# aim-uofa/DiverGen

Measured on AMD Instinct MI355X. Metric: images/sec (node) Swin-L CenterNet2 LVIS 1024px, higher is better.
Workload: dtype bf16; 1 GPU; CenterNet2 Swin-L-22k-384, 1024x1024, 2 images/GPU, 1453 classes, GPU copy-paste + fwd + bwd + fused clip/AdamW/EMA; configs/DiverGen_swinL.yaml; global_batch=2, parallelism=dp1

## Files before the change

### divergen_amd/csrc/gemm_k192.hip

```cpp
#include "gemm_common.h"

namespace {
constexpr int KW_BROWS = 192, KW_KT = 3;
constexpr int KW_BKT = KW_BROWS * 128;
constexpr int KW_B_BYTES = KW_KT * KW_BKT;
template <int AR> struct KwCfg { static constexpr int WAVES = 192 / AR, AKT = AR * 128, A_BYTES = KW_KT * AKT, RI = AR / 16, RQ = AR / 8; };
struct KwParams {
    GemmP g;
    int ntn, row_tiles, wg_per_xcd;
};

template <int MC, int AR>
__global__ __launch_bounds__(KwCfg<AR>::WAVES * 64, 1) void gemm_k192_kernel(KwParams K) {
    constexpr int KW_WAVES = KwCfg<AR>::WAVES, KW_AKT = KwCfg<AR>::AKT, KW_A_BYTES = KwCfg<AR>::A_BYTES, KW_AROWS = AR, RI = KwCfg<AR>::RI,
                  RQ = KwCfg<AR>::RQ;
    GemmP& P = K.g;
    g_fix_mode<MC>(P);
    extern __shared__ __attribute__((aligned(1024))) unsigned char lds_raw[];
    const int tid = threadIdx.x, l = tid & 63;
    const int w = __builtin_amdgcn_readfirstlane(tid >> 6);
    const int c = l & 15, g = l >> 4;
    const int xcd = blockIdx.x & 7, slot = blockIdx.x >> 3;
    const int panel = slot % K.ntn;
    const int full = K.wg_per_xcd / K.ntn, extra = K.wg_per_xcd - full * K.ntn;
    const int groups = 8 * (full + (panel < extra ? 1 : 0));
    const int wave_rank = ((slot / K.ntn) * 8 + xcd) * KW_WAVES + w, wave_count = groups * KW_WAVES;
    const int n0 = panel * KW_BROWS;

    const int rsub = l >> 3;
    const uint32_t lds0 = (uint32_t)(uintptr_t)(DGX_LDS unsigned char*)lds_raw;
    {
        const u32x4 rB = buf_rsrc(P.B, (uint32_t)((int64_t)P.N * P.ldb * 2));
        for (int idx = w; idx < KW_KT * 24; idx += KW_WAVES) {
            const int kt = idx / 24, q = idx - kt * 24;
            const int lc = (l & 7) ^ (((q & 1) << 2) | (rsub >> 1));
            const int n = n0 + 8 * q + rsub;
            const uint32_t voff = (uint32_t)(((int64_t)n * P.ldb + lc * 8) * 2);
            lds_load16(voff, rB, __builtin_amdgcn_readfirstlane(lds0 + (uint32_t)(kt * KW_BKT + q * 1024)), (uint32_t)kt * 128u);
        }
    }
    const uint32_t abase = __builtin_amdgcn_readfirstlane(lds0 + (uint32_t)(KW_B_BYTES + w * KW_A_BYTES));
    const u32x4 rA = buf_rsrc(P.A, (uint32_t)((int64_t)P.M * P.lda * 2));
    uint32_t lcq[RQ];
#pragma unroll
    for (int q = 0; q < RQ; ++q) lcq[q] = (uint32_t)(((l & 7) ^ (((q & 1) << 2) | (rsub >> 1))) * 16);
    auto issue_a = [&](int tile) {
        const int m0 = tile * KW_AROWS;
#pragma unroll
        for (int q = 0; q < RQ; ++q) {
            const int m = m0 + 8 * q + rsub;
            const uint32_t voff = m < P.M ? (uint32_t)((int64_t)m * P.lda * 2) + lcq[q] : BUF_OOB;
#pragma unroll
            for (int kt = 0; kt < KW_KT; ++kt) lds_load16(voff, rA, abase + (uint32_t)(kt * KW_AKT + q * 1024), (uint32_t)kt * 128u);
        }
    };
    u32x2 braw[12];
#pragma unroll
    for (int j = 0; j < 12; ++j) braw[j] = P.bias ? *reinterpret_cast<const u32x2*>(P.bias + n0 + 16 * j + 4 * g) : u32x2{0u, 0u};
    int tile = wave_rank;
    if (tile < K.row_tiles) issue_a(tile);
    wait_vmcnt<0>();
    __syncthreads();

    const int swz = (c >> 1) & 7;
    const uint32_t fa = (uint32_t)(c * 128 + ((g ^ swz) << 4));
    DGX_LDS const unsigned char* pa = lds_opaque((const unsigned char*)lds_raw + KW_B_BYTES + w * KW_A_BYTES + fa);
    DGX_LDS const unsigned char* pa1 = lds_opaque((const unsigned char*)lds_raw + KW_B_BYTES + w * KW_A_BYTES + (fa ^ 64u));
    DGX_LDS const unsigned char* pb = lds_opaque((const unsigned char*)lds_raw + fa);
    DGX_LDS const unsigned char* pb1 = lds_opaque((const unsigned char*)lds_raw + (fa ^ 64u));
    const bool even = (g & 1) == 0;

    int gn[6];
#pragma unroll
    for (int p = 0; p < 6; ++p) gn[p] = n0 + 16 * (2 * p + (even ? 0 : 1)) + 4 * (even ? g : g - 1);
    for (; tile < K.row_tiles; tile += wave_count) {
        u32x4 xpre[MC == 4 ? RI : 1][6];
        if constexpr (MC == 4) {
#pragma unroll
            for (int i = 0; i < RI; ++i) {
                const int gm = tile * KW_AROWS + 16 * i + c;
#pragma unroll
                for (int p = 0; p < 6; ++p) xpre[i][p] = *reinterpret_cast<const u32x4*>(P.aux + (int64_t)(gm < P.M ? gm : 0) * P.ldaux + gn[p]);
            }
        }
        f32x4 acc[RI][12];
#pragma unroll
        for (int i = 0; i < RI; ++i)
#pragma unroll
            for (int j = 0; j < 12; ++j) acc[i][j] = f32x4{0.f, 0.f, 0.f, 0.f};
#pragma unroll
        for (int kt = 0; kt < KW_KT; ++kt)
#pragma unroll
            for (int kh = 0; kh < 2; ++kh) {
                DGX_LDS const unsigned char* a_ = (kh ? pa1 : pa) + kt * KW_AKT;
                DGX_LDS const unsigned char* b_ = (kh ? pb1 : pb) + kt * KW_BKT;
                bf16x8 af[RI];
#pragma unroll
                for (int i = 0; i < RI; ++i) af[i] = *reinterpret_cast<DGX_LDS const bf16x8*>(a_ + 2048 * i);
#pragma unroll
                for (int j = 0; j < 12; ++j) {
                    const bf16x8 b = *reinterpret_cast<DGX_LDS const bf16x8*>(b_ + 2048 * j);
#pragma unroll
                    for (int i = 0; i < RI; ++i) acc[i][j] = mfma16(b, af[i], acc[i][j]);
                }
            }
        const int m0 = tile * KW_AROWS;
        const int next = tile + wave_count;
        wait_lgkm0();
        if (next < K.row_tiles) issue_a(next);
#pragma unroll
        for (int i = 0; i < RI; ++i) {
            const int gm = m0 + 16 * i + c;
            int64_t tok = 0;
            float sc = 1.0f;
            bool ok = gm < P.M;
            if (P.mode == 3 && ok) {
                int b = 0;
                tok = wm_row_token<int64_t, G_ORDERS>(P.map, (int64_t)gm, b);
                ok = tok >= 0;
                if (ok && P.scale) sc = P.scale[b];
            }
            u32x4 y[6];
#pragma unroll
            for (int p = 0; p < 6; ++p) {
                u32x2 pk[2];
#pragma unroll
                for (int h = 0; h < 2; ++h) {
                    const int j = 2 * p + h;
                    const f32x4 a = acc[i][j];
                    float bv[4];
                    g_bias4(braw[j], bv);
                    pk[h] = u32x2{pack_bf2(a[0] + bv[0], a[1] + bv[1]), pack_bf2(a[2] + bv[2], a[3] + bv[3])};
                }
                const u32x2 give = even ? pk[1] : pk[0];
                const u32x2 got = u32x2{(uint32_t)__shfl_xor((int)give[0], 16), (uint32_t)__shfl_xor((int)give[1], 16)};
                y[p] = even ? u32x4{pk[0][0], pk[0][1], got[0], got[1]} : u32x4{got[0], got[1], pk[1][0], pk[1][1]};
            }
            u32x4 xa[6], xb[6];
            if constexpr (MC == 4) {
#pragma unroll
                for (int p = 0; p < 6; ++p) { xa[p] = xpre[i][p]; xb[p] = xa[p]; }
            } else if (P.mode >= 3) {
#pragma unroll
                for (int p = 0; p < 6; ++p) {
                    xa[p] = u32x4{0u, 0u, 0u, 0u}; xb[p] = xa[p];
                    g_epi_prefetch(P, ok ? gm : 0, gn[p], ok ? tok : 0, xa[p], xb[p]);
                }
            }
            if (ok) {
#pragma unroll
                for (int p = 0; p < 6; ++p) g_epi_finish(P, gm, gn[p], y[p], tok, sc, xa[p], xb[p]);
            }
        }
        constexpr int NST = (MC == 1 || MC == 4) ? RI * 6 : MC == 2 ? RI * 12 : -1;
        if (NST >= 0 && m0 + KW_AROWS <= P.M) wait_vmcnt<(NST >= 0 ? NST : 0)>();
        else wait_vmcnt<0>();
    }
}

template <int MC, int AR>
int launch_k192(KwParams& K, hipStream_t st, int grid) {
    static bool once = false;
    const size_t sm = (size_t)KW_B_BYTES + (size_t)KwCfg<AR>::WAVES * KwCfg<AR>::A_BYTES;
    K.row_tiles = (K.g.M + AR - 1) / AR;
    if (!once) {
        (void)hipFuncSetAttribute((const void*)gemm_k192_kernel<MC, AR>, hipFuncAttributeMaxDynamicSharedMemorySize, (int)sm);
        once = true;
    }
    hipLaunchKernelGGL((gemm_k192_kernel<MC, AR>), dim3(grid), dim3(KwCfg<AR>::WAVES * 64), sm, st, K);
    return DGX_OK;
}
}

bool dgx_gemm_k192_takes(const GemmP& P) {
    return P.lda >= 192 && ((uintptr_t)P.A & 15) == 0 && ((uintptr_t)P.B & 15) == 0 && (P.lda & 7) == 0 && (P.ldb & 7) == 0;
}
int dgx_gemm_k192_launch(const GemmP& P0, hipStream_t st) {
    extern int dgx_get_reserved_cus(void);
    KwParams K;
    K.g = P0;
    K.ntn = P0.N / KW_BROWS;
    K.row_tiles = 0;
    K.wg_per_xcd = 32 - dgx_get_reserved_cus() / 8;
    if (P0.K != 192 || K.ntn < 1 || K.wg_per_xcd < K.ntn) return DGX_ERR_UNSUPPORTED;
    const int grid = 8 * K.wg_per_xcd;
    return g_with_mc(g_tail_mc(P0), [&](auto mc) {
        constexpr int v = decltype(mc)::value;
        if constexpr (v == 5) return (int)DGX_ERR_UNSUPPORTED;
        else if constexpr (v <= 1) return launch_k192<1, 32>(K, st, grid);
        else return launch_k192<v, 16>(K, st, grid);
    });
}
```

Measured before the change: 80.81 images/s.

## Load A fragments straight to registers with prefetch, bias in LDS, retune waves

Adds a register-resident A path: each wave loads its A fragments directly from global memory into VGPRs in MFMA layout, double-buffered by prefetching the next tile before the current compute. This drops the LDS staging of A and frees LDS. The bias moves from per-lane registers into a small shared LDS table, and wave counts per workgroup are chosen separately per epilogue mode and panel count. The costs are higher VGPR pressure from the prefetch buffers, and 16-wide A tiles replace 32-wide ones for some modes.

```diff
diff --git a/divergen_amd/csrc/gemm_k192.hip b/divergen_amd/csrc/gemm_k192.hip
--- a/divergen_amd/csrc/gemm_k192.hip
+++ b/divergen_amd/csrc/gemm_k192.hip
@@ -4,16 +4,27 @@
 constexpr int KW_BROWS = 192, KW_KT = 3;
 constexpr int KW_BKT = KW_BROWS * 128;
 constexpr int KW_B_BYTES = KW_KT * KW_BKT;
-template <int AR> struct KwCfg { static constexpr int WAVES = 192 / AR, AKT = AR * 128, A_BYTES = KW_KT * AKT, RI = AR / 16, RQ = AR / 8; };
+template <int AR, int WV> struct KwCfg { static constexpr int WAVES = WV, RI = AR / 16, NA = RI * KW_KT * 2; };
+
+template <int OFF> __device__ __forceinline__ u32x4 kw_load16(uint32_t voff, u32x4 rsrc) {
+    u32x4 r;
+    asm volatile("buffer_load_dwordx4 %0, %1, %2, 0 offen offset:%3" : "=v"(r) : "v"(voff), "s"(rsrc), "n"(OFF) : "memory");
+    return r;
+}
+template <int NA> __device__ __forceinline__ void kw_landed(u32x4 (&a)[NA]) {
+    static_assert(NA == 6 || NA == 12, "fragments per lane");
+    asm volatile("" : "+v"(a[0]), "+v"(a[1]), "+v"(a[2]), "+v"(a[3]), "+v"(a[4]), "+v"(a[5])::"memory");
+    if constexpr (NA == 12) asm volatile("" : "+v"(a[6]), "+v"(a[7]), "+v"(a[8]), "+v"(a[9]), "+v"(a[10]), "+v"(a[11])::"memory");
+}
 struct KwParams {
     GemmP g;
     int ntn, row_tiles, wg_per_xcd;
 };
 
-template <int MC, int AR>
-__global__ __launch_bounds__(KwCfg<AR>::WAVES * 64, 1) void gemm_k192_kernel(KwParams K) {
-    constexpr int KW_WAVES = KwCfg<AR>::WAVES, KW_AKT = KwCfg<AR>::AKT, KW_A_BYTES = KwCfg<AR>::A_BYTES, KW_AROWS = AR, RI = KwCfg<AR>::RI,
-                  RQ = KwCfg<AR>::RQ;
+template <int MC, int AR, int WV, bool LDSA>
+__global__ __launch_bounds__(WV * 64, 1) void gemm_k192_kernel(KwParams K) {
+    constexpr int KW_WAVES = WV, KW_AROWS = AR, RI = KwCfg<AR, WV>::RI, NA = KwCfg<AR, WV>::NA;
+    constexpr int KW_AKT = AR * 128, KW_A_BYTES = KW_KT * KW_AKT, RQ = AR / 8, KW_BIAS_OFF = KW_B_BYTES + (LDSA ? WV * KW_A_BYTES : 0);
     GemmP& P = K.g;
     g_fix_mode<MC>(P);
     extern __shared__ __attribute__((aligned(1024))) unsigned char lds_raw[];
@@ -39,41 +50,63 @@
             lds_load16(voff, rB, __builtin_amdgcn_readfirstlane(lds0 + (uint32_t)(kt * KW_BKT + q * 1024)), (uint32_t)kt * 128u);
         }
     }
-    const uint32_t abase = __builtin_amdgcn_readfirstlane(lds0 + (uint32_t)(KW_B_BYTES + w * KW_A_BYTES));
     const u32x4 rA = buf_rsrc(P.A, (uint32_t)((int64_t)P.M * P.lda * 2));
-    uint32_t lcq[RQ];
-#pragma unroll
-    for (int q = 0; q < RQ; ++q) lcq[q] = (uint32_t)(((l & 7) ^ (((q & 1) << 2) | (rsub >> 1))) * 16);
-    auto issue_a = [&](int tile) {
+    const uint32_t abase =__builtin_amdgcn_readfirstlane(lds0 + (uint32_t)(KW_B_BYTES + w * KW_A_BYTES));
+    auto issue_a_lds = [&](int tile) {
         const int m0 = tile * KW_AROWS;
 #pragma unroll
         for (int q = 0; q < RQ; ++q) {
             const int m = m0 + 8 * q + rsub;
-            const uint32_t voff = m < P.M ? (uint32_t)((int64_t)m * P.lda * 2) + lcq[q] : BUF_OOB;
+            const uint32_t lcq = (uint32_t)(((l & 7) ^ (((q & 1) << 2) | (rsub >> 1))) * 16);
+            const uint32_t voff = m < P.M ? (uint32_t)((int64_t)m * P.lda * 2) + lcq : BUF_OOB;
 #pragma unroll
             for (int kt = 0; kt < KW_KT; ++kt) lds_load16(voff, rA, abase + (uint32_t)(kt * KW_AKT + q * 1024), (uint32_t)kt * 128u);
         }
     };
-    u32x2 braw[12];
-#pragma unroll
-    for (int j = 0; j < 12; ++j) braw[j] = P.bias ? *reinterpret_cast<const u32x2*>(P.bias + n0 + 16 * j + 4 * g) : u32x2{0u, 0u};
+    auto issue_a = [&](int tile, u32x4(&a)[NA]) {
+        static_for<RI>([&](auto i_) {
+            constexpr int i = decltype(i_)::value;
+            const int m = tile * KW_AROWS + 16 * i + c;
+            const uint32_t voff = m < P.M ? (uint32_t)((int64_t)m * P.lda * 2) + (uint32_t)(g * 16) : BUF_OOB;
+            static_for<KW_KT * 2>([&](auto k_) {
+                constexpr int k = decltype(k_)::value;
+                a[i * KW_KT * 2 + k] = kw_load16<k * 64>(voff, rA);
+            });
+        });
+    };
+    if (tid < KW_BROWS / 2)
+        reinterpret_cast<uint32_t*>(lds_raw + KW_BIAS_OFF)[tid] = P.bias ? *reinterpret_cast<const uint32_t*>(P.bias + n0 + 2 * tid) : 0u;
     int tile = wave_rank;
-    if (tile < K.row_tiles) issue_a(tile);
-    wait_vmcnt<0>();
+    u32x4 an[NA];
+    if constexpr (LDSA) {
+        if (tile < K.row_tiles) issue_a_lds(tile);
+        wait_vmcnt<0>();
+    } else {
+        issue_a(tile, an);
+        wait_vmcnt<0>();
+        kw_landed(an);
+    }
     __syncthreads();
 
     const int swz = (c >> 1) & 7;
     const uint32_t fa = (uint32_t)(c * 128 + ((g ^ swz) << 4));
+    DGX_LDS const unsigned char* pb = lds_opaque((const unsigned char*)lds_raw + fa);
+    DGX_LDS const unsigned char* pb1 = lds_opaque((const unsigned char*)lds_raw + (fa ^ 64u));
     DGX_LDS const unsigned char* pa = lds_opaque((const unsigned char*)lds_raw + KW_B_BYTES + w * KW_A_BYTES + fa);
     DGX_LDS const unsigned char* pa1 = lds_opaque((const unsigned char*)lds_raw + KW_B_BYTES + w * KW_A_BYTES + (fa ^ 64u));
-    DGX_LDS const unsigned char* pb = lds_opaque((const unsigned char*)lds_raw + fa);
-    DGX_LDS const unsigned char* pb1 = lds_opaque((const unsigned char*)lds_raw + (fa ^ 64u));
+    DGX_LDS const unsigned char* pbias = lds_opaque((const unsigned char*)lds_raw + KW_BIAS_OFF + 8 * g);
     const bool even = (g & 1) == 0;
 
     int gn[6];
 #pragma unroll
     for (int p = 0; p < 6; ++p) gn[p] = n0 + 16 * (2 * p + (even ? 0 : 1)) + 4 * (even ? g : g - 1);
     for (; tile < K.row_tiles; tile += wave_count) {
+        u32x4 ac[NA];
+        if constexpr (!LDSA) {
+#pragma unroll
+            for (int q = 0; q < NA; ++q) ac[q] = an[q];
+            issue_a(tile + wave_count, an);
+        }
         u32x4 xpre[MC == 4 ? RI : 1][6];
         if constexpr (MC == 4) {
 #pragma unroll
@@ -83,6 +116,7 @@
                 for (int p = 0; p < 6; ++p) xpre[i][p] = *reinterpret_cast<const u32x4*>(P.aux + (int64_t)(gm < P.M ? gm : 0) * P.ldaux + gn[p]);
             }
         }
+        asm volatile("" ::: "memory");
         f32x4 acc[RI][12];
 #pragma unroll
         for (int i = 0; i < RI; ++i)
@@ -92,11 +126,13 @@
         for (int kt = 0; kt < KW_KT; ++kt)
 #pragma unroll
             for (int kh = 0; kh < 2; ++kh) {
-                DGX_LDS const unsigned char* a_ = (kh ? pa1 : pa) + kt * KW_AKT;
                 DGX_LDS const unsigned char* b_ = (kh ? pb1 : pb) + kt * KW_BKT;
                 bf16x8 af[RI];
 #pragma unroll
-                for (int i = 0; i < RI; ++i) af[i] = *reinterpret_cast<DGX_LDS const bf16x8*>(a_ + 2048 * i);
+                for (int i = 0; i < RI; ++i) {
+                    if constexpr (LDSA) af[i] = *reinterpret_cast<DGX_LDS const bf16x8*>((kh ? pa1 : pa) + kt * KW_AKT + 2048 * i);
+                    else af[i] = __builtin_bit_cast(bf16x8, ac[(i * KW_KT + kt) * 2 + kh]);
+                }
 #pragma unroll
                 for (int j = 0; j < 12; ++j) {
                     const bf16x8 b = *reinterpret_cast<DGX_LDS const bf16x8*>(b_ + 2048 * j);
@@ -105,9 +141,10 @@
                 }
             }
         const int m0 = tile * KW_AROWS;
-        const int next = tile + wave_count;
-        wait_lgkm0();
-        if (next < K.row_tiles) issue_a(next);
+        if constexpr (LDSA) {
+            wait_lgkm0();
+            if (tile + wave_count < K.row_tiles) issue_a_lds(tile + wave_count);
+        }
 #pragma unroll
         for (int i = 0; i < RI; ++i) {
             const int gm = m0 + 16 * i + c;
@@ -129,7 +166,7 @@
                     const int j = 2 * p + h;
                     const f32x4 a = acc[i][j];
                     float bv[4];
-                    g_bias4(braw[j], bv);
+                    g_bias4(*reinterpret_cast<DGX_LDS const u32x2*>(pbias + 32 * j), bv);
                     pk[h] = u32x2{pack_bf2(a[0] + bv[0], a[1] + bv[1]), pack_bf2(a[2] + bv[2], a[3] + bv[3])};
                 }
                 const u32x2 give = even ? pk[1] : pk[0];
@@ -155,19 +192,20 @@
         constexpr int NST = (MC == 1 || MC == 4) ? RI * 6 : MC == 2 ? RI * 12 : -1;
         if (NST >= 0 && m0 + KW_AROWS <= P.M) wait_vmcnt<(NST >= 0 ? NST : 0)>();
         else wait_vmcnt<0>();
-    }
-}
-
-template <int MC, int AR>
+        if constexpr (!LDSA) kw_landed(an);
+    }
+}
+
+template <int MC, int AR, int WV, bool LDSA>
 int launch_k192(KwParams& K, hipStream_t st, int grid) {
     static bool once = false;
-    const size_t sm = (size_t)KW_B_BYTES + (size_t)KwCfg<AR>::WAVES * KwCfg<AR>::A_BYTES;
+    const size_t sm = (size_t)KW_B_BYTES + KW_BROWS * 2 + (LDSA ? (size_t)WV * KW_KT * AR * 128 : 0);
     K.row_tiles = (K.g.M + AR - 1) / AR;
     if (!once) {
-        (void)hipFuncSetAttribute((const void*)gemm_k192_kernel<MC, AR>, hipFuncAttributeMaxDynamicSharedMemorySize, (int)sm);
+        (void)hipFuncSetAttribute((const void*)gemm_k192_kernel<MC, AR, WV, LDSA>, hipFuncAttributeMaxDynamicSharedMemorySize, (int)sm);
         once = true;
     }
-    hipLaunchKernelGGL((gemm_k192_kernel<MC, AR>), dim3(grid), dim3(KwCfg<AR>::WAVES * 64), sm, st, K);
+    hipLaunchKernelGGL((gemm_k192_kernel<MC, AR, WV, LDSA>), dim3(grid), dim3(WV * 64), sm, st, K);
     return DGX_OK;
 }
 }
@@ -187,7 +225,8 @@
     return g_with_mc(g_tail_mc(P0), [&](auto mc) {
         constexpr int v = decltype(mc)::value;
         if constexpr (v == 5) return (int)DGX_ERR_UNSUPPORTED;
-        else if constexpr (v <= 1) return launch_k192<1, 32>(K, st, grid);
-        else return launch_k192<v, 16>(K, st, grid);
+        else if constexpr (v <= 1) return K.ntn == 1 ? launch_k192<1, 16, 16, false>(K, st, grid) : launch_k192<1, 32, 6, true>(K, st, grid);
+        else if constexpr (v == 2) return launch_k192<v, 16, 16, false>(K, st, grid);
+        else return launch_k192<v, 16, 12, false>(K, st, grid);
     });
 }
```

After: 80.97 images/s, median of 2. About the same (+0.2%).
